# SobeyMIL/MVOC

Measured on AMD Instinct MI355X. Metric: UNet3D denoising steps/sec, 16x512^2 frames, inversion+compose, higher is better.
Workload: dtype f16

## Files before the change

mvoc_amd/build.py:

```python
import hashlib
import os
import subprocess
import sys

HERE = os.path.dirname(os.path.abspath(__file__))
CSRC = os.path.join(HERE, "csrc")
LIB = os.path.join(HERE, "libmvoc_hip.so")
SOURCES = ["runtime.hip", "gemm.hip", "gemm8.hip", "attention.hip", "tfused.hip", "xslin.hip", "norm.hip", "pnp.hip", "stem.hip", "comm.hip"]
HIPCC = os.environ.get("HIPCC", "/opt/rocm/bin/hipcc")
LAB = os.environ.get("MVOC_BUILD_LAB") == "1"
if LAB:
    LIB = os.path.join(HERE, "libmvoc_hip_lab.so")
VARIANT = os.environ.get("MVOC_BUILD_VARIANT", "")
VARIANT_DEFS = os.environ.get("MVOC_BUILD_DEFS", "").split()
if VARIANT:
    LIB = os.path.join(HERE, f"libmvoc_hip_{VARIANT}.so")
FLAGS = ["--offload-arch=gfx950", "-O3", "-std=c++17", "-fPIC", "-fno-gpu-rdc", "-Wall", "-Wno-unused-function",
         "-ffp-contract=on", "-Rpass-analysis=kernel-resource-usage"]
EXTRA_FLAGS = {"attention.hip": ["-mllvm", "-amdgpu-mfma-vgpr-form"], "gemm.hip": ["-mllvm", "-amdgpu-mfma-vgpr-form"],
               "gemm8.hip": ["-mllvm", "-amdgpu-mfma-vgpr-form", "-falign-loops=64"], "tfused.hip": ["-mllvm", "-amdgpu-mfma-vgpr-form"],
               "xslin.hip": ["-mllvm", "-amdgpu-mfma-vgpr-form"]}


def _digest():
    h = hashlib.sha256()
    for f in sorted(x for x in os.listdir(CSRC) if x.endswith((".hip", ".h"))) + ["../../include/mvoc_hip.h"]:
        with open(os.path.join(CSRC, f), "rb") as fh:
            h.update(fh.read())
    h.update((" ".join(FLAGS + VARIANT_DEFS) + repr(sorted(EXTRA_FLAGS.items()))).encode())
    return h.hexdigest()


def build(force=False, verbose=True):
    stamp = LIB + ".stamp"
    dig = _digest()
    if not force and os.path.exists(LIB) and os.path.exists(stamp) and open(stamp).read() == dig:
        return LIB
    objs = []
    procs = []
    shared = b"".join(open(os.path.join(CSRC, f), "rb").read() for f in sorted(os.listdir(CSRC)) if f.endswith(".h"))
    shared += open(os.path.join(HERE, "..", "include", "mvoc_hip.h"), "rb").read()
    for src in SOURCES:
        obj = os.path.join(CSRC, src.replace(".hip", f".{VARIANT}.o" if VARIANT else (".lab.o" if LAB else ".o")))
        objs.append(obj)
        cmd = [HIPCC, *FLAGS, *(["-DMVOC_PP_LAB"] if LAB else []), *VARIANT_DEFS, *EXTRA_FLAGS.get(src, []), "-c", os.path.join(CSRC, src), "-o", obj]
        od = hashlib.sha256(open(os.path.join(CSRC, src), "rb").read() + shared + " ".join(cmd).encode()).hexdigest()
        ostamp = obj + ".stamp"
        if not force and os.path.exists(obj) and os.path.exists(ostamp) and open(ostamp).read() == od:
            continue
        if verbose:
            print(" ".join(cmd), flush=True)
        procs.append((src, subprocess.Popen(cmd, stdout=subprocess.PIPE, stderr=subprocess.STDOUT, text=True), ostamp, od))
    failed = False
    for src, p, ostamp, od in procs:
        out, _ = p.communicate()
        remarks = "\n".join(l for l in out.splitlines() if "-Rpass-analysis=kernel-resource-usage" in l)
        out = "\n".join(l for l in out.splitlines() if "-Rpass-analysis=kernel-resource-usage" not in l)
        with open(ostamp.replace(".stamp", ".res.txt"), "w") as fh:
            fh.write(remarks + "\n")
        if out.strip() and verbose:
            print(out)
        if p.returncode != 0:
            failed = True
            print(f"hipcc failed on {src}:\n{out}", file=sys.stderr)
        else:
            with open(ostamp, "w") as fh:
                fh.write(od)
    if failed:
        raise RuntimeError("libmvoc_hip.so: compilation failed")
    cmd = [HIPCC, "--offload-arch=gfx950", "-shared", "-fPIC", "-o", LIB, *objs, "-ldl"]
    if verbose:
        print(" ".join(cmd), flush=True)
    subprocess.run(cmd, check=True)
    with open(stamp, "w") as fh:
        fh.write(dig)
    return LIB


if __name__ == "__main__":
    build(force="--force" in sys.argv)
```

mvoc_amd/csrc/attention.hip:

```cpp
#include <stdlib.h>

#include "common.h"

namespace {

typedef __fp16 fp16x4_t __attribute__((__vector_size__(4 * sizeof(__fp16))));
template <int D> struct FlashPitch { static constexpr int K = 2 * D + 16, V = D == 64 ? 192 : 320; };

struct AttnArgs {
  const half_t *q, *k, *v;
  half_t* out;
  long q_bs, q_ts, k_bs, k_ts, v_bs, v_ts, o_bs, o_ts;
  int nbatch, heads, tq, tk, kv_bdiv, causal;
  float scale_log2;
  long v2_off, o2_off;
  int qblocks;
};

__device__ __forceinline__ int vt_slot_group(int key) {
  return ((((key >> 5) * 2 + ((key >> 4) & 1)) * 2) + ((key >> 2) & 1));
}
__device__ __forceinline__ int vt_slot_elem(int key) { return ((key >> 3) & 1) * 4 + (key & 3); }

constexpr float FLASH_THR = 8.0f;
// ... 525 lines not shown
#pragma unroll
  for (int i = 0; i < 4; ++i) {
    const int c = lane + 64 * i;
    const int key = c >> 3, dc = c & 7;
    half8_t vr = zero8;
    if (row_ok(key)) vr = *reinterpret_cast<const half8_t*>(vb + row_px(key) * p.v_ps + (long)row_fr(key) * p.v_ts + dc * 8);
    const int g = (((key >> 4) & 1) * 2) + ((key >> 2) & 1), j = vt_slot_elem(key);
#pragma unroll
    for (int e = 0; e < 8; ++e) {
      const int d = dc * 8 + e;
      *reinterpret_cast<half_t*>(Vs + d * TVPITCH + ((g ^ ((d >> 3) & 3)) * 16) + j * 2) = vr[e];
    }
  }
  f32x16 st;
#pragma unroll
  for (int e = 0; e < 16; ++e) st[e] = 0.f;
  const bool rok = row_ok(r);
  const long koff = row_px(r) * p.k_ps + (long)row_fr(r) * p.k_ts, qoff = row_px(r) * p.q_ps + (long)row_fr(r) * p.q_ts;
#pragma unroll
  for (int s = 0; s < 4; ++s) {
    half8_t kf = zero8, qf = zero8;
    if (rok) {
      kf = *reinterpret_cast<const half8_t*>(kb + koff + 16 * s + 8 * h);
      qf = *reinterpret_cast<const half8_t*>(qb + qoff + 16 * s + 8 * h);
    }
    st = __builtin_amdgcn_mfma_f32_32x32x16_f16(kf, qf, st, 0, 0, 0);
  }
  float mx = -INFINITY;
#pragma unroll
  for (int e = 0; e < 16; ++e) {
    const int key = 8 * (e >> 2) + 4 * h + (e & 3);
    const bool ok = P > 1 ? (key >> logf) == (r >> logf) : key < F;
    const float sv = ok ? st[e] * p.scale_log2 : -INFINITY;
    st[e] = sv;
    mx = fmaxf(mx, sv);
  }
  mx = fmaxf(mx, __shfl_xor(mx, 32));
  float ps = 0.f;
#pragma unroll
  for (int e = 0; e < 16; ++e) {
    const float pv = __builtin_amdgcn_exp2f(st[e] - mx);
    st[e] = pv;
    ps += pv;
  }
  ps += __shfl_xor(ps, 32);
  const float inv = 1.0f / ps;

  __syncthreads();
  f32x16 ot[2];
#pragma unroll
  for (int dt = 0; dt < 2; ++dt)
#pragma unroll
    for (int e = 0; e < 16; ++e) ot[dt][e] = 0.f;
#pragma unroll
  for (int s = 0; s < 2; ++s) {
    half8_t pf;
#pragma unroll
    for (int j = 0; j < 8; ++j) pf[j] = (half_t)st[8 * s + j];
    const int g = s * 2 + h;
#pragma unroll
    for (int dt = 0; dt < 2; ++dt) {
      const int d = 32 * dt + r;
      const half8_t vf = *reinterpret_cast<const half8_t*>(Vs + d * TVPITCH + ((g ^ ((d >> 3) & 3)) * 16));
      ot[dt] = __builtin_amdgcn_mfma_f32_32x32x16_f16(vf, pf, ot[dt], 0, 0, 0);
    }
  }
  if (active && rok) {
    half_t* op = p.out + smp * p.o_bs + (px0 + row_px(r)) * p.o_ps + (long)row_fr(r) * p.o_ts + head * 64;
#pragma unroll
    for (int dt = 0; dt < 2; ++dt)
#pragma unroll
      for (int q = 0; q < 4; ++q) {
        half4_t o;
#pragma unroll
        for (int e = 0; e < 4; ++e) o[e] = (half_t)(ot[dt][q * 4 + e] * inv);
        *reinterpret_cast<half4_t*>(op + 32 * dt + 8 * q + 4 * h) = o;
      }
  }
}

}

static const int g_f3_env = getenv("MVOC_FLASH3") ? atoi(getenv("MVOC_FLASH3")) : -1;

extern "C" int mvoc_flash_attn_f16(const mvoc_attn_desc* d, void* stream) {
  MVOC_REQUIRE(d && d->q && d->k && d->v && d->out, -1, "flash_attn: null operand");
  MVOC_REQUIRE(d->nbatch > 0 && d->heads > 0 && d->tq > 0 && d->tk > 0, -1, "flash_attn: empty problem");
  MVOC_REQUIRE(d->nbatch <= 65535 && d->heads <= 65535, -2, "flash_attn: grid too large");
  MVOC_REQUIRE(d->q_ts % 8 == 0 && d->k_ts % 8 == 0 && d->v_ts % 8 == 0 && d->o_ts % 4 == 0, -2,
               "flash_attn: row strides must keep 16-byte alignment");
  AttnArgs a;
  a.q = (const half_t*)d->q; a.k = (const half_t*)d->k; a.v = (const half_t*)d->v; a.out = (half_t*)d->out;
  a.q_bs = d->q_bs; a.q_ts = d->q_ts; a.k_bs = d->k_bs; a.k_ts = d->k_ts; a.v_bs = d->v_bs; a.v_ts = d->v_ts;
  a.o_bs = d->o_bs; a.o_ts = d->o_ts;
  a.nbatch = d->nbatch; a.heads = d->heads; a.tq = d->tq; a.tk = d->tk; a.kv_bdiv = d->kv_bdiv > 0 ? d->kv_bdiv : 1;
  const int hd = d->head_dim > 0 ? d->head_dim : 64;
  MVOC_REQUIRE(hd == 64 || hd == 96, -2, "flash_attn: head_dim (%d) must be 64 or 96", hd);
  MVOC_REQUIRE(!d->causal || d->tq == d->tk, -2, "flash_attn: the causal form is self-attention (tq == tk)");
  a.causal = d->causal;
  a.scale_log2 = (d->scale > 0.f ? d->scale : (hd == 64 ? 0.125f : 1.0f / sqrtf((float)hd))) * 1.4426950408889634f;
  hipStream_t s = (hipStream_t)stream;
  MvocProfScope prof(MVOC_FAM_FLASH, s, (d->v2 ? 2.0 : 1.0) * 4.0 * d->nbatch * d->heads * (double)d->tq * d->tk * hd);
  a.qblocks = (d->tq + 127) / 128;
  const long nblk = (long)a.qblocks * d->heads * d->nbatch;
  MVOC_REQUIRE(nblk < 0x7fffffffL, -2, "flash_attn: grid too large");
  dim3 grid((unsigned)nblk);
  a.v2_off = a.o2_off = 0;
  MVOC_REQUIRE(d->pipelined >= 0 && d->pipelined <= 2, -1, "flash_attn: pipelined must be 0 (by key count), 1 (never) or 2 (wherever it applies)");
  const int f3_mode = d->pipelined ? d->pipelined - 1 : g_f3_env;
  const bool pipelined = hd == 64 && !d->causal && (f3_mode >= 0 ? f3_mode != 0 : d->tk >= 2048);
  if (d->v2) {
    MVOC_REQUIRE(d->out2 && hd == 64, -2, "flash_attn: the paired form needs out2 and head_dim 64");
    a.v2_off = (const half_t*)d->v2 - a.v;
    a.o2_off = (half_t*)d->out2 - a.out;
    MVOC_REQUIRE(a.v2_off % 8 == 0 && a.o2_off % 4 == 0, -2, "flash_attn: v2 / out2 must keep 16-byte alignment");
    if (pipelined) hipLaunchKernelGGL((flash3_kernel<2>), grid, dim3(256), 0, s, a);
    else hipLaunchKernelGGL((flash_kernel<64, 2>), grid, dim3(256), 0, s, a);
  } else if (hd == 64) {
    if (pipelined) hipLaunchKernelGGL((flash3_kernel<1>), grid, dim3(256), 0, s, a);
    else hipLaunchKernelGGL((flash_kernel<64, 1>), grid, dim3(256), 0, s, a);
  } else {
    hipLaunchKernelGGL((flash_kernel<96, 1>), grid, dim3(256), 0, s, a);
  }
  return mvoc_check_launch("flash_kernel");
}

#ifdef MVOC_F3_STAMPS
extern "C" int mvoc_f3_stamps_read(unsigned long long* host8) {
  return hipMemcpyFromSymbol(host8, HIP_SYMBOL(f3_dbg), sizeof(unsigned long long) * 8) == hipSuccess ? 0 : -1;
}
#endif

extern "C" int mvoc_temporal_attn_f16(const mvoc_tattn_desc* d, void* stream) {
  MVOC_REQUIRE(d && d->q && d->k && d->v && d->out, -1, "temporal_attn: null operand");
  MVOC_REQUIRE(d->nsample > 0 && d->hw > 0 && d->heads > 0, -1, "temporal_attn: empty problem");
  MVOC_REQUIRE(d->frames >= 1 && d->frames <= 32, -2, "temporal_attn: frames (%d) must be in [1, 32]", d->frames);
  MVOC_REQUIRE(d->q_ts % 8 == 0 && d->k_ts % 8 == 0 && d->v_ts % 8 == 0 && d->o_ts % 4 == 0 && d->q_ps % 8 == 0 &&
                   d->k_ps % 8 == 0 && d->v_ps % 8 == 0 && d->o_ps % 4 == 0,
               -2, "temporal_attn: strides must keep 16-byte alignment");
  TAttnArgs a;
  a.q = (const half_t*)d->q; a.k = (const half_t*)d->k; a.v = (const half_t*)d->v; a.out = (half_t*)d->out;
  a.q_bs = d->q_bs; a.q_ps = d->q_ps; a.q_ts = d->q_ts; a.k_bs = d->k_bs; a.k_ps = d->k_ps; a.k_ts = d->k_ts;
  a.v_bs = d->v_bs; a.v_ps = d->v_ps; a.v_ts = d->v_ts; a.o_bs = d->o_bs; a.o_ps = d->o_ps; a.o_ts = d->o_ts;
  a.nsample = d->nsample; a.hw = d->hw; a.heads = d->heads; a.frames = d->frames;
  a.logf = d->frames == 8 ? 3 : d->frames == 16 ? 4 : 5;
  a.logp = d->frames == 8 ? 2 : d->frames == 16 ? 1 : 0;
  a.pgroups = (d->hw + (1 << a.logp) - 1) >> a.logp;
  a.ntask = (long)d->nsample * a.pgroups * d->heads;
  a.scale_log2 = 0.125f * 1.4426950408889634f;
  const long nblk = (a.ntask + 3) / 4;
  MVOC_REQUIRE(nblk < 0x7fffffffL, -2, "temporal_attn: grid too large");
  hipStream_t s = (hipStream_t)stream;
  MvocProfScope prof(MVOC_FAM_TATTN, s, 4.0 * (double)d->nsample * d->hw * d->heads * d->frames * 64 * 2);
  hipLaunchKernelGGL(tattn_kernel, dim3((unsigned)nblk), dim3(256), 0, s, a);
  return mvoc_check_launch("tattn_kernel");
}
```

mvoc_amd/csrc/stem.hip:

```cpp
#include "common.h"

namespace {

__global__ void timestep_embedding_kernel(const float* __restrict__ t, int nb, int dim, half_t* __restrict__ out) {
  const int i = blockIdx.x * blockDim.x + threadIdx.x;
  const int half = dim / 2;
  if (i >= nb * dim) return;
  const int b = i / dim, j = i % dim;
  const int k = j < half ? j : j - half;
  const float freq = expf(-logf(10000.0f) * (float)k / (float)half);
  const float ang = t[b] * freq;
  out[i] = (half_t)(j < half ? cosf(ang) : sinf(ang));
}

__global__ void act_kernel(const half_t* __restrict__ x, half_t* __restrict__ out, long n, int act) {
  const long i = (long)blockIdx.x * blockDim.x + threadIdx.x;
  if (i >= n) return;
  const float v = (float)x[i];
  out[i] = (half_t)(act == MVOC_ACT_SILU ? silu_f(v) : act == MVOC_ACT_GELU ? gelu_erf_f(v) : v);
}

__global__ void add_kernel(const half_t* __restrict__ a, const half_t* __restrict__ b, half_t* __restrict__ out, long n) {
  const long i = (long)blockIdx.x * blockDim.x + threadIdx.x;
  if (i >= n) return;
  out[i] = (half_t)((float)a[i] + (float)b[i]);
}

__global__ void conv3x3_small_kernel(const half_t* __restrict__ x, const half_t* __restrict__ w,
                                     const half_t* __restrict__ bias, half_t* __restrict__ out, int nimg, int h, int wd,
                                     int cin, int cout, int stride, int ho, int wo, int silu) {
  const long i = (long)blockIdx.x * blockDim.x + threadIdx.x;
  const long total = (long)nimg * ho * wo * cout;
  if (i >= total) return;
  const int co = (int)(i % cout);
  long pix = i / cout;
  const int ox = (int)(pix % wo);
  pix /= wo;
  const int oy = (int)(pix % ho);
  const int img = (int)(pix / ho);
  float acc = 0.f;
  for (int ky = 0; ky < 3; ++ky) {
    const int iy = oy * stride + ky - 1;
    if (iy < 0 || iy >= h) continue;
    for (int kx = 0; kx < 3; ++kx) {
      const int ix = ox * stride + kx - 1;
      if (ix < 0 || ix >= wd) continue;
      const half_t* xp = x + (((long)img * h + iy) * wd + ix) * cin;
      const half_t* wp = w + ((long)co * 9 + ky * 3 + kx) * cin;
      for (int c = 0; c < cin; ++c) acc += (float)xp[c] * (float)wp[c];
    }
  }
  float v = r16(acc + (bias ? (float)bias[co] : 0.f));
  if (silu) v = silu_f(v);
  out[i] = (half_t)v;
}

__global__ void avgpool_kernel(const half_t* __restrict__ x, half_t* __restrict__ out, int nimg, int h, int w, int c,
                               int oh, int ow) {
  const long i = (long)blockIdx.x * blockDim.x + threadIdx.x;
  const long total = (long)nimg * oh * ow * c;
  if (i >= total) return;
  const int ch = (int)(i % c);
  long pix = i / c;
  const int ox = (int)(pix % ow);
  pix /= ow;
  const int oy = (int)(pix % oh);
  const int img = (int)(pix / oh);
  const int y0 = (oy * h) / oh, y1 = ((oy + 1) * h + oh - 1) / oh;
  const int x0 = (ox * w) / ow, x1 = ((ox + 1) * w + ow - 1) / ow;
  float s = 0.f;
  for (int y = y0; y < y1; ++y)
    for (int xx = x0; xx < x1; ++xx) s += (float)x[(((long)img * h + y) * w + xx) * c + ch];
  out[i] = (half_t)(s / (float)((y1 - y0) * (x1 - x0)));
}

__global__ void ncfhw_to_tokens_kernel(const half_t* __restrict__ x, half_t* __restrict__ out, int b, int c, int f, int hw,
                                       int ldo, int coff) {
  const long i = (long)blockIdx.x * blockDim.x + threadIdx.x;
  const long total = (long)b * f * hw;
  if (i >= total) return;
  const int p = (int)(i % hw);
  const long bf = i / hw;
  const int fi = (int)(bf % f), bi = (int)(bf / f);
  for (int ch = 0; ch < c; ++ch) out[i * ldo + coff + ch] = x[(((long)bi * c + ch) * f + fi) * hw + p];
}

__global__ void tokens_to_ncfhw_kernel(const half_t* __restrict__ x, half_t* __restrict__ out, int b, int c, int f, int hw,
                                       int ld) {
  const long i = (long)blockIdx.x * blockDim.x + threadIdx.x;
  const long total = (long)b * c * f * hw;
  if (i >= total) return;
  const int p = (int)(i % hw);
  long r = i / hw;
  const int fi = (int)(r % f);
  r /= f;
  const int ch = (int)(r % c);
  const int bi = (int)(r / c);
  out[i] = x[(((long)bi * f + fi) * hw + p) * ld + ch];
}

struct Enc4Params {
  half_t ln_g[4], ln_b[4], wq[32], wk[32], wv[32], wo[32], bo[4], w1[64], b1[16], w2[64], b2[4];
};

__device__ __forceinline__ void enc4_ln(const half_t* xp, const Enc4Params& P, float* y) {
  float v[4], mean = 0.f;
#pragma unroll
  for (int c = 0; c < 4; ++c) { v[c] = (float)xp[c]; mean += v[c]; }
// ... 72 lines not shown
  float ff[16];
#pragma unroll
  for (int o = 0; o < 16; ++o) {
    float s = 0.f;
#pragma unroll
    for (int c = 0; c < 4; ++c) s += h1[c] * (float)P.w1[o * 4 + c];
    ff[o] = r16(gelu_erf_f(r16(s + (float)P.b1[o])));
  }
#pragma unroll
  for (int c = 0; c < 4; ++c) {
    float s = 0.f;
#pragma unroll
    for (int o = 0; o < 16; ++o) s += ff[o] * (float)P.w2[c * 16 + o];
    out[idx * ldo + coff + c] = (half_t)(r16(s + (float)P.b2[c]) + h1[c]);
  }
}

__global__ void delay_kernel(long ticks) {
  const long t0 = __builtin_amdgcn_s_memrealtime();
  while ((long)__builtin_amdgcn_s_memrealtime() - t0 < ticks) __builtin_amdgcn_s_sleep(32);
}

inline unsigned nblk(long n, int bs = 256) { return (unsigned)((n + bs - 1) / bs); }

__global__ __launch_bounds__(256) void clip_patches_kernel(const half_t* __restrict__ x, half_t* __restrict__ out, int size, int patch,
                                                           int kpad, long total) {
  const long i = (long)blockIdx.x * 256 + threadIdx.x;
  if (i >= total) return;
  const int g = size / patch;
  const int k = (int)(i % kpad);
  const long row = i / kpad;
  half_t v = (half_t)0.f;
  if (k < 3 * patch * patch) {
    const int c = k / (patch * patch), py = (k / patch) % patch, px = k % patch;
    const int gx = (int)(row % g), gy = (int)((row / g) % g);
    const long b = row / ((long)g * g);
    v = x[((b * 3 + c) * size + gy * patch + py) * (long)size + gx * patch + px];
  }
  out[i] = v;
}

__global__ __launch_bounds__(256) void clip_embed_kernel(const half_t* __restrict__ table, const int* __restrict__ ids,
                                                         const half_t* __restrict__ cls, const half_t* __restrict__ pos,
                                                         half_t* __restrict__ out, int T, int c8n, long total) {
  const long i = (long)blockIdx.x * 256 + threadIdx.x;
  if (i >= total) return;
  const int c8 = (int)(i % c8n);
  const long row = i / c8n;
  const int t = (int)(row % T);
  const half_t* src;
  if (ids) src = table + ((long)ids[row] * c8n + c8) * 8;
  else if (t == 0) src = cls + c8 * 8;
  else src = table + (((row / T) * (T - 1) + t - 1) * c8n + c8) * 8;
  const half8_t a = *reinterpret_cast<const half8_t*>(src);
  const half8_t b = *reinterpret_cast<const half8_t*>(pos + ((long)t * c8n + c8) * 8);
  half8_t o;
#pragma unroll
  for (int e = 0; e < 8; ++e) o[e] = (half_t)((float)a[e] + (float)b[e]);
  reinterpret_cast<half8_t*>(out)[i] = o;
}

}

extern "C" int mvoc_timestep_embedding_f16(const float* t_dev, int32_t nb, int32_t dim, void* out, void* stream) {
  MVOC_REQUIRE(t_dev && out && nb > 0 && dim > 0 && dim % 2 == 0, -1, "timestep_embedding: bad args");
  hipStream_t s = (hipStream_t)stream;
  MvocProfScope prof(MVOC_FAM_MISC, s, 2.0 * nb * dim);
  hipLaunchKernelGGL(timestep_embedding_kernel, dim3(nblk((long)nb * dim)), dim3(256), 0, s, t_dev, nb, dim, (half_t*)out);
  return mvoc_check_launch("timestep_embedding_kernel");
}

extern "C" int mvoc_act_f16(const void* x, void* out, int64_t n, int32_t act, void* stream) {
  MVOC_REQUIRE(x && out && n > 0, -1, "act: bad args");
  hipStream_t s = (hipStream_t)stream;
  MvocProfScope prof(MVOC_FAM_MISC, s, 4.0 * n);
  hipLaunchKernelGGL(act_kernel, dim3(nblk(n)), dim3(256), 0, s, (const half_t*)x, (half_t*)out, (long)n, act);
  return mvoc_check_launch("act_kernel");
}

extern "C" int mvoc_add_f16(const void* a, const void* b, void* out, int64_t n, void* stream) {
  MVOC_REQUIRE(a && b && out && n > 0, -1, "add: bad args");
  hipStream_t s = (hipStream_t)stream;
  MvocProfScope prof(MVOC_FAM_MISC, s, 6.0 * n);
  hipLaunchKernelGGL(add_kernel, dim3(nblk(n)), dim3(256), 0, s, (const half_t*)a, (const half_t*)b, (half_t*)out, (long)n);
  return mvoc_check_launch("add_kernel");
}

extern "C" int mvoc_conv3x3_small_f16(const void* x, const void* w, const void* bias, void* out, int32_t nimg, int32_t h,
                                      int32_t wd, int32_t cin, int32_t cout, int32_t stride, int32_t silu, void* stream) {
  MVOC_REQUIRE(x && w && out && nimg > 0 && h > 0 && wd > 0 && cin > 0 && cout > 0 && (stride == 1 || stride == 2), -1,
               "conv3x3_small: bad args");
  const int ho = (h + 2 - 3) / stride + 1, wo = (wd + 2 - 3) / stride + 1;
  const long total = (long)nimg * ho * wo * cout;
  hipStream_t s = (hipStream_t)stream;
  MvocProfScope prof(MVOC_FAM_MISC, s, 2.0 * ((double)nimg * h * wd * cin + total));
  hipLaunchKernelGGL(conv3x3_small_kernel, dim3(nblk(total)), dim3(256), 0, s, (const half_t*)x, (const half_t*)w,
                     (const half_t*)bias, (half_t*)out, nimg, h, wd, cin, cout, stride, ho, wo, silu);
  return mvoc_check_launch("conv3x3_small_kernel");
}

__global__ void conv1x1_small_kernel(const half_t* __restrict__ x, const half_t* __restrict__ w, const half_t* __restrict__ bias,
                                     half_t* __restrict__ out, long rows, int cin, int cout) {
  const long i = (long)blockIdx.x * blockDim.x + threadIdx.x;
  if (i >= rows * cout) return;
  const int co = (int)(i % cout);
  const long r = i / cout;
  float acc = 0.f;
  for (int c = 0; c < cin; ++c) acc += (float)x[r * cin + c] * (float)w[co * cin + c];
  out[i] = (half_t)(acc + (bias ? (float)bias[co] : 0.f));
}

__global__ void image_to_tokens_kernel(const half_t* __restrict__ x, half_t* __restrict__ out, int n, int c, int hw) {
  const long i = (long)blockIdx.x * blockDim.x + threadIdx.x;
  if (i >= (long)n * hw * c) return;
  const int ch = (int)(i % c);
  const long px = i / c;
  const int img = (int)(px / hw), p = (int)(px % hw);
  out[i] = x[((long)img * c + ch) * hw + p];
}
__global__ void tokens_to_image_kernel(const half_t* __restrict__ x, half_t* __restrict__ out, int n, int c, int hw, int ld) {
  const long i = (long)blockIdx.x * blockDim.x + threadIdx.x;
  if (i >= (long)n * c * hw) return;
  const int p = (int)(i % hw);
  const long t = i / hw;
  const int ch = (int)(t % c), img = (int)(t / c);
  out[i] = x[((long)img * hw + p) * ld + ch];
}

__global__ void gaussian_sample_kernel(const half_t* __restrict__ mean, const half_t* __restrict__ logvar,
                                       const half_t* __restrict__ noise, half_t* __restrict__ out, long n) {
  const long i = (long)blockIdx.x * blockDim.x + threadIdx.x;
  if (i >= n) return;
  const float lv = fminf(fmaxf((float)logvar[i], -30.0f), 20.0f);
  const float sd = r16(expf(r16(0.5f * lv)));
  out[i] = (half_t)((float)mean[i] + r16(sd * (float)noise[i]));
}
__global__ void scale_kernel(const half_t* __restrict__ x, half_t* __restrict__ out, long n, float s) {
  const long i = (long)blockIdx.x * blockDim.x + threadIdx.x;
  if (i >= n) return;
  float p = s * (float)x[i];
  asm volatile("" : "+v"(p));
  out[i] = (half_t)p;
}

extern "C" int mvoc_gaussian_sample_f16(const void* mean, const void* logvar, const void* noise, void* out, int64_t n, void* stream) {
  MVOC_REQUIRE(mean && logvar && noise && out && n > 0, -1, "gaussian_sample: bad args");
  hipStream_t s = (hipStream_t)stream;
  MvocProfScope prof(MVOC_FAM_MISC, s, 8.0 * n);
  hipLaunchKernelGGL(gaussian_sample_kernel, dim3(nblk(n)), dim3(256), 0, s, (const half_t*)mean, (const half_t*)logvar,
                     (const half_t*)noise, (half_t*)out, (long)n);
  return mvoc_check_launch("gaussian_sample_kernel");
}

extern "C" int mvoc_clip_patches_f16(const void* pixels, void* out, int32_t nimg, int32_t size, int32_t patch, int32_t kpad,
                                     void* stream) {
  MVOC_REQUIRE(pixels && out && nimg > 0 && patch > 0 && size > 0 && size % patch == 0 && kpad >= 3 * patch * patch, -1,
               "clip_patches: bad args");
  const long total = (long)nimg * (size / patch) * (size / patch) * kpad;
  hipStream_t s = (hipStream_t)stream;
  MvocProfScope prof(MVOC_FAM_MISC, s, 4.0 * total);
  hipLaunchKernelGGL(clip_patches_kernel, dim3(nblk(total)), dim3(256), 0, s, (const half_t*)pixels, (half_t*)out, size, patch, kpad, total);
  return mvoc_check_launch("clip_patches_kernel");
}

extern "C" int mvoc_clip_embed_f16(const void* table, const int32_t* ids, const void* cls, const void* pos, void* out, int64_t rows,
                                   int32_t t, int32_t c, void* stream) {
  MVOC_REQUIRE(table && pos && out && rows > 0 && t > 0 && rows % t == 0 && c > 0 && c % 8 == 0 && (ids || cls), -1,
// ... 160 lines not shown
```

mvoc_amd/csrc/xslin.hip:

```cpp
#include <stdlib.h>

#include "common.h"

namespace {

struct XsArgs {
  const half_t* x;
  const half_t* wp;
  const half_t* resid;
  half_t* out;
  long M;
  int N, n_store, ldo, ldr, act, normalize;
  float eps;
  unsigned long long* stamps;
  int lab;
  long set_rows;
  long set_bytes;
};

#ifdef MVOC_PP_LAB
#define XS_STAMP(t) asm volatile("s_memtime %0\n\ts_waitcnt lgkmcnt(0)" : "=s"(t)::"memory")
#define XS_ACC(slot, a, b) (acc_t[slot] += (b) - (a))
#else
#define XS_STAMP(t) do { } while (0)
// ... 220 lines not shown
        for (int e = 0; e < 16; ++e) acc[g][e] = 0.f;
      run_stage(acc);
      half2_t hv[RG][8];
#pragma unroll
      for (int q = 0; q < 4; ++q) {
        const f32x4 cvl = cvec4(cslot, 8 * q + 4 * h);
#pragma unroll
        for (int g = 0; g < RG; ++g) {
          hv[g][2 * q] = half2_t{(half_t)(acc[g][4 * q] + cvl[0]), (half_t)(acc[g][4 * q + 1] + cvl[1])};
          hv[g][2 * q + 1] = half2_t{(half_t)(acc[g][4 * q + 2] + cvl[2]), (half_t)(acc[g][4 * q + 3] + cvl[3])};
        }
      }
#pragma unroll
      for (int g = 0; g < RG; ++g)
#pragma unroll
        for (int e = 0; e < 16; ++e) acc[g][e] = 0.f;
      run_stage(acc);
#pragma unroll
      for (int g = 0; g < RG; ++g) {
        unsigned pk[4][2];
#pragma unroll
        for (int q = 0; q < 4; ++q) {
          const f32x4 cgt = cvec4(cslot, 8 * q + 4 * h);
          half_t o[4];
#pragma unroll
          for (int e = 0; e < 4; ++e) {
            const float gv = r16(acc[g][4 * q + e] + cgt[e]);
            o[e] = (half_t)((float)hv[g][2 * q + (e >> 1)][e & 1] * r16(gelu_fast_f(gv)));
          }
          const half2_t lo = {o[0], o[1]}, hi = {o[2], o[3]};
          pk[q][0] = __builtin_bit_cast(unsigned, lo);
          pk[q][1] = __builtin_bit_cast(unsigned, hi);
        }
        store_tile(pk, 16 * t, t + 1, g);
      }
    }
  } else {
    for (int t = 0; t < T; ++t) {
      f32x16 acc[RG];
#pragma unroll
      for (int g = 0; g < RG; ++g)
#pragma unroll
        for (int e = 0; e < 16; ++e) acc[g][e] = 0.f;
      run_stage(acc);
      if (p.resid) wait_resid(t);
#pragma unroll
      for (int g = 0; g < RG; ++g) {
        unsigned pk[4][2];
#pragma unroll
        for (int q = 0; q < 4; ++q) {
          const f32x4 cv = cvec4(cslot, 8 * q + 4 * h);
          half_t o[4];
#pragma unroll
          for (int e = 0; e < 4; ++e) {
            float v = r16(acc[g][4 * q + e] + cv[e]);
            if constexpr (ACT == MVOC_ACT_SILU) v = r16(silu_f(v));
            else if constexpr (ACT == MVOC_ACT_GELU) v = r16(gelu_fast_f(v));
            o[e] = (half_t)v;
          }
          const half2_t lo = {o[0], o[1]}, hi = {o[2], o[3]};
          pk[q][0] = __builtin_bit_cast(unsigned, lo);
          pk[q][1] = __builtin_bit_cast(unsigned, hi);
        }
        store_tile(pk, 32 * t, t, g);
      }
      if (RG == 2 && p.resid && t + 1 < T) {
        asm volatile("s_waitcnt lgkmcnt(0)" ::: "memory");
        issue_resid(t + 1);
      }
    }
  }
#ifdef MVOC_PP_LAB
  XS_STAMP(ta);
  XS_ACC(3, te, ta);
  if (p.stamps && blockIdx.x == 0 && wave == 0 && lane == 0) {
    for (int i = 0; i < 4; ++i) p.stamps[i] = acc_t[i];
    p.stamps[4] = ta - tstart;
    p.stamps[5] = (unsigned long long)T;
  }
#endif
}

}

extern "C" int mvoc_xs_linear_f16(const mvoc_xs_desc* d, void* stream) {
  MVOC_REQUIRE(d && d->x && d->wp && d->out, -1, "xs_linear: null operand");
  MVOC_REQUIRE(d->m > 0 && d->n > 0 && d->n % 32 == 0, -1, "xs_linear: m > 0, n %% 32 == 0");
  MVOC_REQUIRE(d->act >= MVOC_ACT_NONE && d->act <= MVOC_ACT_GELU, -1, "xs_linear: bad act %d", d->act);
  MVOC_REQUIRE(!(d->resid && d->act == MVOC_ACT_GEGLU), -2, "xs_linear: no residual with GEGLU");
  MVOC_REQUIRE(d->k == 64 || d->k == 128 || d->k == 320, -2, "xs_linear: k (%d) must be 64, 128 or 320", d->k);
  MVOC_REQUIRE(d->act != MVOC_ACT_GEGLU || d->n % 64 == 0, -2, "xs_linear: GEGLU needs n %% 64 == 0");
  const int ns = d->n_store > 0 ? d->n_store : (d->act == MVOC_ACT_GEGLU ? d->n / 2 : d->n);
  MVOC_REQUIRE(ns > (d->act == MVOC_ACT_GEGLU ? d->n / 2 : d->n) - 32, -2, "xs_linear: n_store may only trim the last 32-channel tile");
  MVOC_REQUIRE(ns % 8 == 0 && d->ldo % 8 == 0 && ((uintptr_t)d->out & 15) == 0 &&
                   (d->resid == nullptr || (d->ldr % 8 == 0 && ((uintptr_t)d->resid & 15) == 0)),
               -2, "xs_linear: outputs / residual must be 16-byte addressable per 8 channels");
  XsArgs a;
  a.x = (const half_t*)d->x; a.wp = (const half_t*)d->wp;
  a.resid = (const half_t*)d->resid; a.out = (half_t*)d->out;
  a.M = d->m; a.N = d->n; a.n_store = ns; a.ldo = d->ldo; a.ldr = d->ldr; a.act = d->act; a.normalize = d->normalize; a.eps = d->ln_eps;
  static const int force_rg = getenv("MVOC_XS_RG") ? atoi(getenv("MVOC_XS_RG")) : 0;
  const int rg = force_rg ? force_rg : (d->m >= 131072 && d->k == 320 ? 2 : 1);
  a.stamps = nullptr;
  a.lab = 0;
  a.set_rows = d->wp_set_rows;
  a.set_bytes = (long)(d->n / 32) * (d->k / 16 + 1) * 1024;
  MVOC_REQUIRE(d->wp_set_rows >= 0 && (d->wp_set_rows == 0 || (d->wp_set_rows % (128 * rg) == 0 && d->m % d->wp_set_rows == 0)), -2,
               "xs_linear: wp_set_rows (%ld) must be a multiple of the %d rows of a block and divide m", (long)d->wp_set_rows, 128 * rg);
#ifdef MVOC_PP_LAB
  if (const char* e = getenv("MVOC_XS_STAMPS")) a.stamps = (unsigned long long*)strtoull(e, nullptr, 10);
  a.lab = getenv("MVOC_XS_LAB") ? atoi(getenv("MVOC_XS_LAB")) : 0;
#endif
  const long nblk = (d->m + 128 * rg - 1) / (128 * rg);
  MVOC_REQUIRE(nblk < 0x7fffffffL, -2, "xs_linear: grid too large");
  hipStream_t s = (hipStream_t)stream;
  MvocProfScope prof(MVOC_FAM_GEMM, s, 2.0 * (double)d->m * d->n * d->k);
  const dim3 grid((unsigned)nblk), blk(256);
#define XS_LAUNCH(NK_, RG_)                                                                                        \
  do {                                                                                                             \
    if (d->act == MVOC_ACT_GEGLU) hipLaunchKernelGGL((xslin_kernel<NK_, RG_, MVOC_ACT_GEGLU>), grid, blk, 0, s, a);  \
    else if (d->act == MVOC_ACT_SILU) hipLaunchKernelGGL((xslin_kernel<NK_, RG_, MVOC_ACT_SILU>), grid, blk, 0, s, a); \
    else if (d->act == MVOC_ACT_GELU) hipLaunchKernelGGL((xslin_kernel<NK_, RG_, MVOC_ACT_GELU>), grid, blk, 0, s, a); \
    else hipLaunchKernelGGL((xslin_kernel<NK_, RG_, MVOC_ACT_NONE>), grid, blk, 0, s, a);                          \
  } while (0)
  if (d->k == 320 && rg == 2) XS_LAUNCH(20, 2);
  else if (d->k == 320) XS_LAUNCH(20, 1);
  else if (d->k == 128 && rg == 2) XS_LAUNCH(8, 2);
  else if (d->k == 128) XS_LAUNCH(8, 1);
  else if (rg == 2) XS_LAUNCH(4, 2);
  else XS_LAUNCH(4, 1);
#undef XS_LAUNCH
  return mvoc_check_launch("xslin_kernel");
}
```

Baseline: 21.79.

## Add short-key cross-attention kernel, persistent weight-stationary linear, vectorized add

Adds a cross-attention kernel for head_dim 64 with at most 192 keys. It loads all K/V into LDS once per block and loops over many 32-query groups, with a split count sized to the CU count. It also adds a persistent weight-stationary 320x320 linear that keeps the weights in registers and streams x tiles through a triple-buffered global-to-LDS pipeline. Both paths are on by default and can be turned off with environment variables. The elementwise add kernel now uses 8-wide vector loads and a grid-stride loop with a capped grid; the new kernels add complexity and their own correctness constraints.

```diff
diff --git a/mvoc_amd/build.py b/mvoc_amd/build.py
--- a/mvoc_amd/build.py
+++ b/mvoc_amd/build.py
@@ -6,7 +6,7 @@
 HERE = os.path.dirname(os.path.abspath(__file__))
 CSRC = os.path.join(HERE, "csrc")
 LIB = os.path.join(HERE, "libmvoc_hip.so")
-SOURCES = ["runtime.hip", "gemm.hip", "gemm8.hip", "attention.hip", "tfused.hip", "xslin.hip", "norm.hip", "pnp.hip", "stem.hip", "comm.hip"]
+SOURCES = ["runtime.hip", "gemm.hip", "gemm8.hip", "attention.hip", "xattn.hip", "tfused.hip", "xslin.hip", "wslin.hip", "norm.hip", "pnp.hip", "stem.hip", "comm.hip"]
 HIPCC = os.environ.get("HIPCC", "/opt/rocm/bin/hipcc")
 LAB = os.environ.get("MVOC_BUILD_LAB") == "1"
 if LAB:
@@ -19,7 +19,8 @@
          "-ffp-contract=on", "-Rpass-analysis=kernel-resource-usage"]
 EXTRA_FLAGS = {"attention.hip": ["-mllvm", "-amdgpu-mfma-vgpr-form"], "gemm.hip": ["-mllvm", "-amdgpu-mfma-vgpr-form"],
                "gemm8.hip": ["-mllvm", "-amdgpu-mfma-vgpr-form", "-falign-loops=64"], "tfused.hip": ["-mllvm", "-amdgpu-mfma-vgpr-form"],
-               "xslin.hip": ["-mllvm", "-amdgpu-mfma-vgpr-form"]}
+               "xslin.hip": ["-mllvm", "-amdgpu-mfma-vgpr-form"], "wslin.hip": ["-mllvm", "-amdgpu-mfma-vgpr-form"],
+               "xattn.hip": ["-mllvm", "-amdgpu-mfma-vgpr-form"]}
 
 
 def _digest():
diff --git a/mvoc_amd/csrc/attention.hip b/mvoc_amd/csrc/attention.hip
--- a/mvoc_amd/csrc/attention.hip
+++ b/mvoc_amd/csrc/attention.hip
@@ -631,6 +631,9 @@
 }
 
 static const int g_f3_env = getenv("MVOC_FLASH3") ? atoi(getenv("MVOC_FLASH3")) : -1;
+bool mvoc_xattn_applies(const mvoc_attn_desc* d);
+int mvoc_xattn_launch(const mvoc_attn_desc* d, float scale_log2, hipStream_t s);
+static const int g_xattn_env = getenv("MVOC_XATTN") ? atoi(getenv("MVOC_XATTN")) : 1;
 
 extern "C" int mvoc_flash_attn_f16(const mvoc_attn_desc* d, void* stream) {
   MVOC_REQUIRE(d && d->q && d->k && d->v && d->out, -1, "flash_attn: null operand");
@@ -666,6 +669,7 @@
     if (pipelined) hipLaunchKernelGGL((flash3_kernel<2>), grid, dim3(256), 0, s, a);
     else hipLaunchKernelGGL((flash_kernel<64, 2>), grid, dim3(256), 0, s, a);
   } else if (hd == 64) {
+    if (d->pipelined == 0 && g_f3_env < 0 && g_xattn_env != 0 && mvoc_xattn_applies(d)) return mvoc_xattn_launch(d, a.scale_log2, s);
     if (pipelined) hipLaunchKernelGGL((flash3_kernel<1>), grid, dim3(256), 0, s, a);
     else hipLaunchKernelGGL((flash_kernel<64, 1>), grid, dim3(256), 0, s, a);
   } else {
diff --git a/mvoc_amd/csrc/stem.hip b/mvoc_amd/csrc/stem.hip
--- a/mvoc_amd/csrc/stem.hip
+++ b/mvoc_amd/csrc/stem.hip
@@ -20,10 +20,18 @@
   out[i] = (half_t)(act == MVOC_ACT_SILU ? silu_f(v) : act == MVOC_ACT_GELU ? gelu_erf_f(v) : v);
 }
 
-__global__ void add_kernel(const half_t* __restrict__ a, const half_t* __restrict__ b, half_t* __restrict__ out, long n) {
-  const long i = (long)blockIdx.x * blockDim.x + threadIdx.x;
-  if (i >= n) return;
-  out[i] = (half_t)((float)a[i] + (float)b[i]);
+__global__ __launch_bounds__(256) void add_kernel(const half_t* __restrict__ a, const half_t* __restrict__ b, half_t* __restrict__ out, long n) {
+  const long i0 = (long)blockIdx.x * blockDim.x + threadIdx.x, step = (long)gridDim.x * blockDim.x;
+  const bool vec = ((reinterpret_cast<uintptr_t>(a) | reinterpret_cast<uintptr_t>(b) | reinterpret_cast<uintptr_t>(out)) & 15) == 0;
+  const long nv = vec ? n >> 3 : 0;
+  for (long i = i0; i < nv; i += step) {
+    const half8_t x = reinterpret_cast<const half8_t*>(a)[i], y = reinterpret_cast<const half8_t*>(b)[i];
+    half8_t o;
+#pragma unroll
+    for (int e = 0; e < 8; ++e) o[e] = (half_t)((float)x[e] + (float)y[e]);
+    reinterpret_cast<half8_t*>(out)[i] = o;
+  }
+  for (long i = nv * 8 + i0; i < n; i += step) out[i] = (half_t)((float)a[i] + (float)b[i]);
 }
 
 __global__ void conv3x3_small_kernel(const half_t* __restrict__ x, const half_t* __restrict__ w,
@@ -262,7 +270,8 @@
   MVOC_REQUIRE(a && b && out && n > 0, -1, "add: bad args");
   hipStream_t s = (hipStream_t)stream;
   MvocProfScope prof(MVOC_FAM_MISC, s, 6.0 * n);
-  hipLaunchKernelGGL(add_kernel, dim3(nblk(n)), dim3(256), 0, s, (const half_t*)a, (const half_t*)b, (half_t*)out, (long)n);
+  const long nb = (n / 8 + 255) / 256;
+  hipLaunchKernelGGL(add_kernel, dim3((unsigned)(nb < 1 ? 1 : nb > 4096 ? 4096 : nb)), dim3(256), 0, s, (const half_t*)a, (const half_t*)b, (half_t*)out, (long)n);
   return mvoc_check_launch("add_kernel");
 }
 
diff --git a/mvoc_amd/csrc/wslin.hip b/mvoc_amd/csrc/wslin.hip
--- /dev/null
+++ b/mvoc_amd/csrc/wslin.hip
@@ -0,0 +1,182 @@
+#include <stdlib.h>
+
+#include <type_traits>
+
+#include "common.h"
+
+namespace {
+
+struct WsArgs {
+  const half_t* x;
+  const half_t* wp;
+  half_t* out;
+  long M;
+  int ldo;
+  long set_rows, set_bytes;
+};
+
+template <int N_>
+__device__ __forceinline__ void ws_wait() {
+  asm volatile("s_waitcnt vmcnt(%0)" ::"n"(N_) : "memory");
+}
+__device__ __forceinline__ void ws_wait_n(int n) {
+  switch (n) {
+    case 0: ws_wait<0>(); break;   case 1: ws_wait<1>(); break;   case 2: ws_wait<2>(); break;   case 3: ws_wait<3>(); break;
+    case 4: ws_wait<4>(); break;   case 5: ws_wait<5>(); break;   case 6: ws_wait<6>(); break;   case 7: ws_wait<7>(); break;
+    case 8: ws_wait<8>(); break;   case 9: ws_wait<9>(); break;   case 10: ws_wait<10>(); break; case 11: ws_wait<11>(); break;
+    default: ws_wait<12>(); break;
+  }
+}
+
+template <int NK, int NT>
+__global__ __launch_bounds__(NT * 64) void wslin_kernel(const WsArgs p) {
+  constexpr int K = NK * 16;
+  constexpr int NSLOT = 3;
+  constexpr int TX = NK * 1024;
+  constexpr int SLOT = TX;
+  constexpr int XPW = (NK + NT - 1) / NT;
+  static_assert(NK % NT == 0, "the x pieces divide evenly over the waves (the counted waits assume it)");
+  __shared__ __attribute__((aligned(1024))) char smem[NSLOT * SLOT + NT * 128];
+  float* cst = reinterpret_cast<float*>(smem + NSLOT * SLOT);
+  const int tid = threadIdx.x, lane = tid & 63;
+  const int wave = __builtin_amdgcn_readfirstlane(tid >> 6);
+  const int r = lane & 31, h = lane >> 5;
+  const long ntile = (p.M + 31) / 32;
+  const long t_begin = ntile * blockIdx.x / gridDim.x, t_end = ntile * (blockIdx.x + 1) / gridDim.x;
+  constexpr int D = XPW;
+
+  auto row_in_tile = [&](long tt) -> int {
+    const long left = p.M - 32 * tt;
+    return left >= 32 ? r : (r < (int)left ? r : (int)left - 1);
+  };
+  auto issue_tile = [&](long tt, int slot) {
+    char* sx = smem + slot * SLOT;
+    const int rr = row_in_tile(tt);
+    const half_t* xb = p.x + tt * 32 * K;
+#pragma unroll
+    for (int i = 0; i < XPW; ++i) {
+      const int j = wave * XPW + i;
+      __builtin_amdgcn_global_load_lds((const __attribute__((address_space(1))) void*)(xb + (rr * K + 16 * j + 8 * h)),
+                                       (__attribute__((address_space(3))) void*)(sx + j * 1024), 16, 0, 0);
+    }
+  };
+
+  long t = t_begin;
+  while (t < t_end) {
+    long seg_end = t_end;
+    const char* wset = reinterpret_cast<const char*>(p.wp);
+    if (p.set_rows > 0) {
+      const long set = (32 * t) / p.set_rows;
+      wset += set * p.set_bytes;
+      const long lim = ((set + 1) * p.set_rows + 31) / 32;
+      seg_end = lim < t_end ? lim : t_end;
+    }
+    half8_t wf[NK];
+    {
+      const char* wt = wset + (size_t)wave * (NK + 1) * 1024 + lane * 16;
+#pragma unroll
+      for (int s = 0; s < NK; ++s) wf[s] = *reinterpret_cast<const half8_t*>(wt + s * 1024);
+    }
+    if (lane < 32) cst[wave * 32 + lane] = reinterpret_cast<const float*>(wset + ((size_t)wave * (NK + 1) + NK) * 1024)[lane];
+    asm volatile("s_waitcnt vmcnt(0) lgkmcnt(0)" ::: "memory");
+#pragma unroll
+    for (int s = 0; s < NK; ++s) asm volatile("" : "+v"(wf[s]));
+    const long n = seg_end - t;
+    int issued = 0, mark0 = 0, mark1 = 0, mark2 = 0;
+    if (n > 0) { issue_tile(t, 0); issued += D; mark0 = issued; }
+    if (n > 1) { issue_tile(t + 1, 1); issued += D; mark1 = issued; }
+
+    auto tile_body = [&](auto SL_, long i) {
+      constexpr int SL = decltype(SL_)::value, SN = (SL + 2) % NSLOT;
+      ws_wait_n(issued - (SL == 0 ? mark0 : SL == 1 ? mark1 : mark2));
+      __builtin_amdgcn_sched_barrier(0);
+      __builtin_amdgcn_s_barrier();
+      __builtin_amdgcn_sched_barrier(0);
+      if (i + 2 < n) {
+        issue_tile(t + i + 2, SN);
+        issued += D;
+        (SN == 0 ? mark0 : SN == 1 ? mark1 : mark2) = issued;
+      }
+      const char* sx = smem + SL * SLOT;
+      f32x16 acc;
+#pragma unroll
+      for (int e = 0; e < 16; ++e) acc[e] = 0.f;
+      {
+        const char* xl = sx + lane * 16;
+        constexpr int PD = 6;
+        half8_t xf[PD];
+#pragma unroll
+        for (int s = 0; s < PD; ++s) xf[s] = *reinterpret_cast<const half8_t*>(xl + s * 1024);
+        __builtin_amdgcn_sched_group_barrier(0x100, PD + (0), 0);
+#pragma unroll
+        for (int s = 0; s < NK; ++s) {
+          acc = __builtin_amdgcn_mfma_f32_32x32x16_f16(wf[s], xf[s % PD], acc, 0, 0, 0);
+          if (s + PD < NK) xf[s % PD] = *reinterpret_cast<const half8_t*>(xl + (s + PD) * 1024);
+          __builtin_amdgcn_sched_group_barrier(0x008, 1, 0);
+          __builtin_amdgcn_sched_group_barrier(0x100, 1, 0);
+        }
+      }
+      unsigned pk[4][2];
+#pragma unroll
+      for (int q = 0; q < 4; ++q) {
+        const f32x4 cvq = *reinterpret_cast<const f32x4*>(cst + wave * 32 + 8 * q + 4 * h);
+        half_t o[4];
+#pragma unroll
+        for (int e = 0; e < 4; ++e) o[e] = (half_t)r16(acc[4 * q + e] + cvq[e]);
+        const half2_t lo = {o[0], o[1]}, hi = {o[2], o[3]};
+        pk[q][0] = __builtin_bit_cast(unsigned, lo);
+        pk[q][1] = __builtin_bit_cast(unsigned, hi);
+      }
+#pragma unroll
+      for (int qq = 0; qq < 4; qq += 2)
+#pragma unroll
+        for (int w2 = 0; w2 < 2; ++w2) {
+          const auto sw = __builtin_amdgcn_permlane32_swap(pk[qq][w2], pk[qq + 1][w2], false, false);
+          pk[qq][w2] = sw[0];
+          pk[qq + 1][w2] = sw[1];
+        }
+      half_t* ob = p.out + (t + i) * 32 * p.ldo;
+      const int oo = row_in_tile(t + i) * p.ldo + 32 * wave + 8 * h;
+#pragma unroll
+      for (int j = 0; j < 2; ++j) {
+        const uint4 v = {pk[2 * j][0], pk[2 * j][1], pk[2 * j + 1][0], pk[2 * j + 1][1]};
+        *reinterpret_cast<uint4*>(ob + (oo + 16 * j)) = v;
+      }
+      issued += 2;
+    };
+    for (long i = 0; i < n; i += 3) {
+      tile_body(std::integral_constant<int, 0>{}, i);
+      if (i + 1 < n) tile_body(std::integral_constant<int, 1>{}, i + 1);
+      if (i + 2 < n) tile_body(std::integral_constant<int, 2>{}, i + 2);
+    }
+    asm volatile("s_waitcnt vmcnt(0) lgkmcnt(0)" ::: "memory");
+    __builtin_amdgcn_s_barrier();
+    t = seg_end;
+  }
+}
+
+}
+
+__attribute__((visibility("hidden"))) bool mvoc_wslin_applies(const mvoc_xs_desc* d) {
+  return d->n == 320 && d->k == 320 && d->act == MVOC_ACT_NONE && d->normalize == 0 && d->resid == nullptr &&
+         (d->n_store == 0 || d->n_store == d->n) && d->ldo % 8 == 0 && ((uintptr_t)d->out & 15) == 0 && ((uintptr_t)d->x & 15) == 0 &&
+         ((uintptr_t)d->wp & 15) == 0 && (d->wp_set_rows == 0 || (d->wp_set_rows > 0 && d->wp_set_rows % 32 == 0 && d->m % d->wp_set_rows == 0));
+}
+
+__attribute__((visibility("hidden"))) int mvoc_wslin_launch(const mvoc_xs_desc* d, hipStream_t s) {
+  MVOC_REQUIRE(mvoc_wslin_applies(d), -2, "ws_linear: n = k = 320, plain epilogue, no residual, 16-byte addressable operands");
+  WsArgs a;
+  a.x = (const half_t*)d->x; a.wp = (const half_t*)d->wp; a.out = (half_t*)d->out;
+  a.M = d->m; a.ldo = d->ldo;
+  a.set_rows = d->wp_set_rows;
+  a.set_bytes = (long)(d->n / 32) * (d->k / 16 + 1) * 1024;
+  const long ntile = (d->m + 31) / 32;
+  static const int cus = [] {
+    int dev = 0, n = 256;
+    if (hipGetDevice(&dev) != hipSuccess || hipDeviceGetAttribute(&n, hipDeviceAttributeMultiprocessorCount, dev) != hipSuccess) n = 256;
+    return n > 0 ? n : 256;
+  }();
+  const long nblk = ntile < cus ? ntile : cus;
+  hipLaunchKernelGGL((wslin_kernel<20, 10>), dim3((unsigned)nblk), dim3(640), 0, s, a);
+  return mvoc_check_launch("wslin_kernel");
+}
diff --git a/mvoc_amd/csrc/xattn.hip b/mvoc_amd/csrc/xattn.hip
--- /dev/null
+++ b/mvoc_amd/csrc/xattn.hip
@@ -0,0 +1,257 @@
+#include <stdlib.h>
+
+#include <type_traits>
+
+#include "common.h"
+
+namespace {
+
+typedef __fp16 fp16x4_t __attribute__((__vector_size__(4 * sizeof(__fp16))));
+typedef float f32x2 __attribute__((ext_vector_type(2)));
+
+constexpr int XA_KPITCH = 144, XA_VPITCH = 192;
+constexpr int XA_MAXK = 192;
+constexpr float XA_THR = 8.0f;
+
+struct XAttnArgs {
+  const half_t *q, *k, *v;
+  half_t* out;
+  long q_bs, q_ts, k_bs, k_ts, v_bs, v_ts, o_bs, o_ts;
+  int nbatch, heads, tq, tk, kv_bdiv;
+  float scale_log2;
+  int gpb;
+  int splits;
+};
+
+__device__ __forceinline__ float xa_xhalf_max(float x) {
+  const unsigned u = __builtin_bit_cast(unsigned, x);
+  const auto sw = __builtin_amdgcn_permlane32_swap(u, u, false, false);
+  return fmaxf(__builtin_bit_cast(float, (unsigned)sw[0]), __builtin_bit_cast(float, (unsigned)sw[1]));
+}
+
+template <int NW>
+__global__ __launch_bounds__(NW * 64, NW / 2) void xattn_kernel(const XAttnArgs p) {
+  constexpr int D = 64, NTH = NW * 64;
+  constexpr int NIT = (XA_MAXK * 8 + NTH - 1) / NTH;
+  __shared__ __attribute__((aligned(16))) char smem[XA_MAXK * (XA_KPITCH + XA_VPITCH)];
+  char* Ks = smem;
+  char* Vs = smem + XA_MAXK * XA_KPITCH;
+  const int tid = threadIdx.x, lane = tid & 63;
+  const int wave = __builtin_amdgcn_readfirstlane(tid >> 6);
+  const int r = lane & 31, h = lane >> 5;
+  const unsigned logical = xcd_remap(blockIdx.x, gridDim.x);
+  const int sp = (int)(logical % (unsigned)p.splits), pair = (int)(logical / (unsigned)p.splits);
+  const int head = pair % p.heads, ent = pair / p.heads;
+  const int ntiles = (p.tk + 63) / 64;
+
+  {
+    const char* kb = reinterpret_cast<const char*>(p.k + (long)ent * p.k_bs + head * D);
+    const char* vb = reinterpret_cast<const char*>(p.v + (long)ent * p.v_bs + head * D);
+    const unsigned k_rb = (unsigned)p.k_ts * 2u, v_rb = (unsigned)p.v_ts * 2u;
+    const int nchunk = ntiles * 64 * 8;
+    half8_t kreg[NIT], vreg[NIT];
+#pragma unroll
+    for (int i = 0; i < NIT; ++i) {
+      const int c = tid + i * NTH;
+      if (c < nchunk) {
+        const unsigned row = (unsigned)min(c >> 3, p.tk - 1), dc = (unsigned)(c & 7);
+        kreg[i] = *reinterpret_cast<const half8_t*>(kb + (size_t)row * k_rb + dc * 16u);
+        vreg[i] = *reinterpret_cast<const half8_t*>(vb + (size_t)row * v_rb + dc * 16u);
+      }
+    }
+#pragma unroll
+    for (int i = 0; i < NIT; ++i) {
+      const int c = tid + i * NTH;
+      if (c < nchunk) {
+        *reinterpret_cast<half8_t*>(Ks + (c >> 3) * XA_KPITCH + (c & 7) * 16) = kreg[i];
+        *reinterpret_cast<half8_t*>(Vs + (c >> 3) * XA_VPITCH + (c & 7) * 16) = vreg[i];
+      }
+    }
+  }
+  __syncthreads();
+
+  const int b0 = ent * p.kv_bdiv;
+  const int nb_e = min(p.kv_bdiv, p.nbatch - b0);
+  const int G = nb_e * p.gpb;
+  const int g0 = (int)((long)G * sp / p.splits), gn = (int)((long)G * (sp + 1) / p.splits) - g0;
+  const int w0 = g0 + (int)((long)gn * wave / NW), w1 = g0 + (int)((long)gn * (wave + 1) / NW);
+  auto qload = [&](int g, half8_t(&qd)[4]) {
+    const int b = b0 + g / p.gpb, q0 = (g % p.gpb) * 32;
+    const half_t* qb = p.q + (long)b * p.q_bs + head * D;
+    int lane_e = tid;
+    asm volatile("" : "+v"(lane_e));
+    const unsigned qo = (unsigned)min(q0 + (lane_e & 31), p.tq - 1) * (unsigned)p.q_ts + 8u * (unsigned)((lane_e >> 5) & 1);
+#pragma unroll
+    for (int s = 0; s < 4; ++s) qd[s] = *reinterpret_cast<const half8_t*>(qb + qo + 16 * s);
+  };
+  half8_t qf[4];
+  if (w0 < w1) qload(w0, qf);
+
+  for (int g = w0; g < w1; ++g) {
+    const bool more = g + 1 < w1;
+
+    f32x16 ot[2];
+#pragma unroll
+    for (int dt = 0; dt < 2; ++dt)
+#pragma unroll
+      for (int e = 0; e < 16; ++e) ot[dt][e] = 0.f;
+    float mrun = -INFINITY, lrun = 0.f;
+
+    auto tile = [&](auto H_, const int kt) {
+      constexpr int H = decltype(H_)::value;
+      const char* Kt = Ks + kt * 64 * XA_KPITCH;
+      const char* Vt = Vs + kt * 64 * XA_VPITCH;
+      f32x16 st[H];
+#pragma unroll
+      for (int t = 0; t < H; ++t) {
+#pragma unroll
+        for (int e = 0; e < 16; ++e) st[t][e] = 0.f;
+#pragma unroll
+        for (int s = 0; s < 4; ++s) {
+          const half8_t kf = *reinterpret_cast<const half8_t*>(Kt + (32 * t + r) * XA_KPITCH + (16 * s + 8 * h) * 2);
+          st[t] = __builtin_amdgcn_mfma_f32_32x32x16_f16(kf, qf[s], st[t], 0, 0, 0);
+        }
+      }
+      if (more && kt == ntiles - 1) qload(g + 1, qf);
+      if (__builtin_amdgcn_readfirstlane((kt == ntiles - 1) && (p.tk & 63))) {
+#pragma unroll
+        for (int t = 0; t < H; ++t)
+#pragma unroll
+          for (int e = 0; e < 16; ++e)
+            if (kt * 64 + 32 * t + 8 * (e >> 2) + 4 * h + (e & 3) >= p.tk) st[t][e] = -INFINITY;
+      }
+      float mx = st[0][0];
+#pragma unroll
+      for (int t = 0; t < H; ++t)
+#pragma unroll
+        for (int e = 0; e < 16; ++e) mx = fmaxf(mx, st[t][e]);
+      mx = xa_xhalf_max(mx);
+      if (__any((mx - mrun) * p.scale_log2 > XA_THR)) {
+        const float mnew = fmaxf(mrun, mx);
+        const float alpha = __builtin_amdgcn_exp2f((mrun - mnew) * p.scale_log2);
+        mrun = mnew;
+        lrun *= alpha;
+#pragma unroll
+        for (int dt = 0; dt < 2; ++dt)
+#pragma unroll
+          for (int e = 0; e < 16; ++e) ot[dt][e] *= alpha;
+      }
+      const f32x2 sc2 = {p.scale_log2, p.scale_log2}, mc2 = {-mrun * p.scale_log2, -mrun * p.scale_log2};
+#pragma unroll
+      for (int t = 0; t < H; ++t)
+#pragma unroll
+        for (int e = 0; e < 16; e += 2) {
+          const f32x2 a = __builtin_elementwise_fma(f32x2{st[t][e], st[t][e + 1]}, sc2, mc2);
+          st[t][e] = __builtin_amdgcn_exp2f(a[0]);
+          st[t][e + 1] = __builtin_amdgcn_exp2f(a[1]);
+        }
+#pragma unroll
+      for (int t = 0; t < H; ++t)
+#pragma unroll
+        for (int s = 0; s < 2; ++s) {
+          if (__builtin_amdgcn_readfirstlane(kt * 64 + 32 * t + 16 * s >= p.tk)) continue;
+          half8_t pf;
+#pragma unroll
+          for (int j = 0; j < 8; ++j) pf[j] = (half_t)st[t][8 * s + j];
+#pragma unroll
+          for (int j = 0; j < 4; ++j) lrun = __builtin_amdgcn_fdot2(half2_t{pf[2 * j], pf[2 * j + 1]}, half2_t{(half_t)1.f, (half_t)1.f}, lrun, false);
+          const int krow = 32 * t + 16 * s + 4 * h + ((lane & 15) >> 2);
+#pragma unroll
+          for (int dt = 0; dt < 2; ++dt) {
+            const char* va = Vt + krow * XA_VPITCH + (32 * dt + 16 * ((lane >> 4) & 1) + 4 * (lane & 3)) * 2;
+            const fp16x4_t lo = __builtin_amdgcn_ds_read_tr16_b64_v4f16((__attribute__((address_space(3))) fp16x4_t*)va);
+            const fp16x4_t hi = __builtin_amdgcn_ds_read_tr16_b64_v4f16((__attribute__((address_space(3))) fp16x4_t*)(va + 8 * XA_VPITCH));
+            half8_t vf;
+#pragma unroll
+            for (int e = 0; e < 4; ++e) {
+              vf[e] = (half_t)lo[e];
+              vf[4 + e] = (half_t)hi[e];
+            }
+            ot[dt] = __builtin_amdgcn_mfma_f32_32x32x16_f16(vf, pf, ot[dt], 0, 0, 0);
+          }
+        }
+    };
+    for (int kt = 0; kt < ntiles; ++kt) {
+      if (__builtin_amdgcn_readfirstlane(kt * 64 + 32 < p.tk)) tile(std::integral_constant<int, 2>{}, kt);
+      else tile(std::integral_constant<int, 1>{}, kt);
+    }
+
+    const unsigned lu = __builtin_bit_cast(unsigned, lrun);
+    const auto lsw = __builtin_amdgcn_permlane32_swap(lu, lu, false, false);
+    const float ltot = __builtin_bit_cast(float, (unsigned)lsw[0]) + __builtin_bit_cast(float, (unsigned)lsw[1]);
+    const float inv = 1.0f / ltot;
+    const int b = b0 + g / p.gpb, q0 = (g % p.gpb) * 32;
+    unsigned pk[2][4][2];
+#pragma unroll
+    for (int dt = 0; dt < 2; ++dt)
+#pragma unroll
+      for (int q = 0; q < 4; ++q) {
+        half_t o[4];
+#pragma unroll
+        for (int e = 0; e < 4; ++e) o[e] = (half_t)(ot[dt][q * 4 + e] * inv);
+        const half2_t lo = {o[0], o[1]}, hi = {o[2], o[3]};
+        pk[dt][q][0] = __builtin_bit_cast(unsigned, lo);
+        pk[dt][q][1] = __builtin_bit_cast(unsigned, hi);
+      }
+#pragma unroll
+    for (int dt = 0; dt < 2; ++dt)
+#pragma unroll
+      for (int qq = 0; qq < 4; qq += 2)
+#pragma unroll
+        for (int w2 = 0; w2 < 2; ++w2) {
+          const auto sw = __builtin_amdgcn_permlane32_swap(pk[dt][qq][w2], pk[dt][qq + 1][w2], false, false);
+          pk[dt][qq][w2] = sw[0];
+          pk[dt][qq + 1][w2] = sw[1];
+        }
+    int lane_e = tid;
+    asm volatile("" : "+v"(lane_e));
+    const int r_e = lane_e & 31, h_e = (lane_e >> 5) & 1;
+    if (q0 + r_e < p.tq) {
+      half_t* ob = p.out + (long)b * p.o_bs + head * D;
+      const unsigned oo = (unsigned)(q0 + r_e) * (unsigned)p.o_ts + 8u * (unsigned)h_e;
+#pragma unroll
+      for (int dt = 0; dt < 2; ++dt)
+#pragma unroll
+        for (int j = 0; j < 2; ++j) {
+          const uint4 v = {pk[dt][2 * j][0], pk[dt][2 * j][1], pk[dt][2 * j + 1][0], pk[dt][2 * j + 1][1]};
+          *reinterpret_cast<uint4*>(ob + oo + 32 * dt + 16 * j) = v;
+        }
+    }
+  }
+}
+
+constexpr int XA_NW = 8;
+
+}
+
+__attribute__((visibility("hidden"))) bool mvoc_xattn_applies(const mvoc_attn_desc* d) {
+  const int hd = d->head_dim > 0 ? d->head_dim : 64, bdiv = d->kv_bdiv > 0 ? d->kv_bdiv : 1;
+  return hd == 64 && !d->causal && d->v2 == nullptr && d->tk <= XA_MAXK && d->o_ts % 8 == 0 && d->o_bs % 8 == 0 &&
+         ((uintptr_t)d->out & 15) == 0 && (long)d->tq * d->q_ts < (1L << 30) && (long)d->tq * d->o_ts < (1L << 30) && d->q_ts >= 0 &&
+         d->o_ts >= 0 && (bdiv > 1 || (d->tq + 127) / 128 >= 4);
+}
+
+__attribute__((visibility("hidden"))) int mvoc_xattn_launch(const mvoc_attn_desc* d, float scale_log2, hipStream_t s) {
+  MVOC_REQUIRE(mvoc_xattn_applies(d), -2, "xattn: head dim 64, no mask, one V, tk <= %d", XA_MAXK);
+  XAttnArgs a;
+  a.q = (const half_t*)d->q; a.k = (const half_t*)d->k; a.v = (const half_t*)d->v; a.out = (half_t*)d->out;
+  a.q_bs = d->q_bs; a.q_ts = d->q_ts; a.k_bs = d->k_bs; a.k_ts = d->k_ts; a.v_bs = d->v_bs; a.v_ts = d->v_ts;
+  a.o_bs = d->o_bs; a.o_ts = d->o_ts;
+  a.nbatch = d->nbatch; a.heads = d->heads; a.tq = d->tq; a.tk = d->tk; a.kv_bdiv = d->kv_bdiv > 0 ? d->kv_bdiv : 1;
+  a.scale_log2 = scale_log2;
+  a.gpb = (d->tq + 31) / 32;
+  static const int cus = [] {
+    int dev = 0, n = 256;
+    if (hipGetDevice(&dev) != hipSuccess || hipDeviceGetAttribute(&n, hipDeviceAttributeMultiprocessorCount, dev) != hipSuccess) n = 256;
+    return n > 0 ? n : 256;
+  }();
+  const long entries = ((long)d->nbatch + a.kv_bdiv - 1) / a.kv_bdiv, pairs = entries * d->heads;
+  const long groups = (long)(a.kv_bdiv < d->nbatch ? a.kv_bdiv : d->nbatch) * a.gpb;
+  long splits = 2L * cus / pairs;
+  if (splits > groups / XA_NW) splits = groups / XA_NW;
+  if (splits < 1) splits = 1;
+  a.splits = (int)splits;
+  MVOC_REQUIRE(pairs * splits < 0x7fffffffL && groups < 0x7fffffffL, -2, "xattn: grid too large");
+  hipLaunchKernelGGL((xattn_kernel<XA_NW>), dim3((unsigned)(pairs * splits)), dim3(XA_NW * 64), 0, s, a);
+  return mvoc_check_launch("xattn_kernel");
+}
diff --git a/mvoc_amd/csrc/xslin.hip b/mvoc_amd/csrc/xslin.hip
--- a/mvoc_amd/csrc/xslin.hip
+++ b/mvoc_amd/csrc/xslin.hip
@@ -326,6 +326,10 @@
 }
 
 }
+
+bool mvoc_wslin_applies(const mvoc_xs_desc* d);
+int mvoc_wslin_launch(const mvoc_xs_desc* d, hipStream_t s);
+static const int g_wslin_env = getenv("MVOC_WSLIN") ? atoi(getenv("MVOC_WSLIN")) : 1;
 
 extern "C" int mvoc_xs_linear_f16(const mvoc_xs_desc* d, void* stream) {
   MVOC_REQUIRE(d && d->x && d->wp && d->out, -1, "xs_linear: null operand");
@@ -359,6 +363,7 @@
   MVOC_REQUIRE(nblk < 0x7fffffffL, -2, "xs_linear: grid too large");
   hipStream_t s = (hipStream_t)stream;
   MvocProfScope prof(MVOC_FAM_GEMM, s, 2.0 * (double)d->m * d->n * d->k);
+  if (g_wslin_env != 0 && mvoc_wslin_applies(d)) return mvoc_wslin_launch(d, s);
   const dim3 grid((unsigned)nblk), blk(256);
 #define XS_LAUNCH(NK_, RG_)                                                                                        \
   do {                                                                                                             \
```

Result: no change. 21.82 (median of 6 runs) (+0.1%).
